# aurelienwaite/SparkNet

Hardware: AMD Instinct MI355X
Metric: images/sec AlexNet training (227x227) at 1/2/4/8 MI355X; scaling efficiency (higher is better)
Workload: dtype bf16; 1 GPU; model=caffenet (bvlc_reference_caffenet / AlexNet), global_batch=256, per_gpu_batch=256, parallelism=dp1, algorithm=local SGD, tau=50, RCCL all-reduce weight averaging, hipgraph=True, streams=3, feed_group=2, fused_input_fold=True, fp8_layers=0, fp8_wgrad=False

## Files before the change

### csrc/kernels/softmax.hip

```cpp
#include "common.h"

#define FLT_MIN_ 1.175494351e-38f

__global__ void softmax_xent_fwd(const bf16_t* __restrict__ x, const float* __restrict__ labels,
                                 float* __restrict__ prob, float* __restrict__ row_loss, float* __restrict__ row_valid,
                                 int M, int C, int has_ignore, int ignore_label) {
  const int lane = threadIdx.x & 63;
  const int row = blockIdx.x * (blockDim.x >> 6) + (threadIdx.x >> 6);
  if (row >= M) return;
  const bf16_t* xr = x + (long long)row * C;
  float m = -INFINITY;
  for (int c = lane; c < C; c += 64) m = fmaxf(m, bf2f(xr[c]));
  m = wave_max(m);
  float s = 0.f;
  for (int c = lane; c < C; c += 64) s += __expf(bf2f(xr[c]) - m);
  s = wave_sum(s);
  const float inv = 1.f / s;
  float* pr = prob + (long long)row * C;
  for (int c = lane; c < C; c += 64) pr[c] = __expf(bf2f(xr[c]) - m) * inv;
  if (lane == 0) {
    int lab = (int)labels[row];
    bool valid = !(has_ignore && lab == ignore_label);
    float nll = 0.f;
    if (valid) {
      float p = __expf(bf2f(xr[min(max(lab, 0), C - 1)]) - m) * inv;
      nll = -__logf(fmaxf(p, FLT_MIN_));
    }
    row_loss[row] = nll;
    row_valid[row] = valid ? 1.f : 0.f;
  }
}

__global__ void xent_reduce(const float* __restrict__ row_loss, const float* __restrict__ row_valid, int M,
                            int normalize, float outer_num, float* __restrict__ out_loss, float* __restrict__ out_norm) {
  __shared__ float ls[16], vs[16];
  float l = 0.f, v = 0.f;
  for (int i = threadIdx.x; i < M; i += blockDim.x) {
    l += row_loss[i];
    v += row_valid[i];
  }
  l = wave_sum(l);
  v = wave_sum(v);
  if ((threadIdx.x & 63) == 0) {
    ls[threadIdx.x >> 6] = l;
    vs[threadIdx.x >> 6] = v;
  }
  __syncthreads();
// ... 4 lines not shown
    norm = fmaxf(norm, 1.f);
    out_loss[0] = L / norm;
    out_norm[0] = norm;
  }
}

extern "C" int sn_softmax_xent_fwd(const bf16_t* x, const float* labels, float* prob, float* row_loss,
                                   float* row_valid, float* out_loss, float* out_norm, long long M, long long C,
                                   long long has_ignore, long long ignore_label, long long normalize,
                                   long long outer_num, hipStream_t st) {
  const int rows_per_block = 4;
  hipLaunchKernelGGL(softmax_xent_fwd, dim3((unsigned)((M + rows_per_block - 1) / rows_per_block)), dim3(256), 0, st, x,
                     labels, prob, row_loss, row_valid, (int)M, (int)C, (int)has_ignore, (int)ignore_label);
  hipLaunchKernelGGL(xent_reduce, dim3(1), dim3(1024), 0, st, row_loss, row_valid, (int)M, (int)normalize,
                     (float)outer_num, out_loss, out_norm);
  return SN_CHECK_LAUNCH();
}

__global__ void softmax_xent_bwd(const float* __restrict__ prob, const float* __restrict__ labels,
                                 const float* __restrict__ loss_weight, const float* __restrict__ norm,
                                 bf16_t* __restrict__ dx, int M, int C, int has_ignore, int ignore_label) {
  const long long total = (long long)M * C;
  const float scale = loss_weight[0] / norm[0];
  for (long long i = blockIdx.x * (long long)blockDim.x + threadIdx.x; i < total; i += (long long)gridDim.x * blockDim.x) {
    const int row = (int)(i / C), c = (int)(i - (long long)row * C);
    const int lab = (int)labels[row];
    float g = 0.f;
    if (!(has_ignore && lab == ignore_label)) g = (prob[i] - (c == lab ? 1.f : 0.f)) * scale;
    dx[i] = f2bf(g);
  }
// ... 78 lines not shown
```

### csrc/kernels/solver.hip

```cpp
#include "common.h"

enum { H_LR = 0, H_MOM, H_WD, H_CLIP, H_NORM, H_DELTA, H_MOM2, H_RMS, H_CORR, H_T, H_SUMSQ = 15 };

SN_DEV void chunk_grad(const float* __restrict__ g, long long o, const long long* __restrict__ src, int cid, int i,
                       float* G) {
  const long long sp = src ? src[4 * cid] : 0;
  if (sp == 0) {
    const float4 gv = *reinterpret_cast<const float4*>(g + o);
    G[0] = gv.x; G[1] = gv.y; G[2] = gv.z; G[3] = gv.w;
    return;
  }
  const float* sl = reinterpret_cast<const float*>(sp);
  const long long ss = src[4 * cid + 1], es = src[4 * cid + 3];
  const int splits = (int)src[4 * cid + 2];
  G[0] = G[1] = G[2] = G[3] = 0.f;
  if (splits >= 16) {
    if (es == 1) {
      const float* p = sl + i;
      for (int l = 0; l < 16; ++l) {
        float P[4] = {0.f, 0.f, 0.f, 0.f};
        int s = l;
        for (; s + 48 < splits; s += 64) {
          float4 v[4];
#pragma unroll
// ... 187 lines not shown
  dim3 grid((unsigned)(grid_limit > 0 && grid_limit < nchunks ? grid_limit : nchunks));
  bool sh = shadow != nullptr;
  const int n = (int)nchunks;
  switch (kind) {
    case 0: launch_kind<0>(l1, clip, sh, grid, st, w, g, h0, h1, shadow, chunk_pos, chunk_mult, hyper, n, chunk_src); break;
    case 1: launch_kind<1>(l1, clip, sh, grid, st, w, g, h0, h1, shadow, chunk_pos, chunk_mult, hyper, n, chunk_src); break;
    case 2: launch_kind<2>(l1, clip, sh, grid, st, w, g, h0, h1, shadow, chunk_pos, chunk_mult, hyper, n, chunk_src); break;
    case 3: launch_kind<3>(l1, clip, sh, grid, st, w, g, h0, h1, shadow, chunk_pos, chunk_mult, hyper, n, chunk_src); break;
    case 4: launch_kind<4>(l1, clip, sh, grid, st, w, g, h0, h1, shadow, chunk_pos, chunk_mult, hyper, n, chunk_src); break;
    case 5: launch_kind<5>(l1, clip, sh, grid, st, w, g, h0, h1, shadow, chunk_pos, chunk_mult, hyper, n, chunk_src); break;
    default: return 8;
  }
  return SN_CHECK_LAUNCH();
}

__global__ void scale_shadow(float* __restrict__ w, bf16_t* __restrict__ shadow, long long n, long long n4,
                             float scale) {
  const long long stride = (long long)gridDim.x * blockDim.x;
  for (long long i = blockIdx.x * (long long)blockDim.x + threadIdx.x; i < n4; i += stride) {
    float4 v = reinterpret_cast<float4*>(w)[i];
    v.x *= scale; v.y *= scale; v.z *= scale; v.w *= scale;
    reinterpret_cast<float4*>(w)[i] = v;
    if (shadow) reinterpret_cast<uint2*>(shadow)[i] = make_uint2(pack2(v.x, v.y), pack2(v.z, v.w));
  }
  for (long long i = 4 * n4 + blockIdx.x * (long long)blockDim.x + threadIdx.x; i < n; i += stride) {
    const float v = w[i] * scale;
    w[i] = v;
    if (shadow) shadow[i] = f2bf(v);
  }
}
// ... 10 lines not shown
```

### sparknet_amd/core/net.py

```python
from __future__ import annotations

import logging
from dataclasses import dataclass, field

import torch

from .. import ops, proto
from .blob import Blob
from .filler import fill
from .layer import Layer, Param, create_layer

log = logging.getLogger("sparknet_amd.net")

PARAM_ALIGN = 64


@dataclass
class NetContext:
    device: torch.device
    dtype: torch.dtype
    phase: int
    seed: int = 1701
    gen: torch.Generator = field(default=None)
    rng_state: torch.Tensor = field(default=None)
# ... 367 lines not shown
            elif prev is not None and prev.numel() == p.count:
                p.data.copy_(prev.reshape(p.shape).to(dev))
        for p in self.params:
            if p.owner is not None:
                r = p.owner
                p.offset = r.offset
                p.data = r.data.view(p.shape)
                p.diff = r.diff.view(p.shape)
                p.compute = r.compute.view(p.shape)
        self.sync_compute()

    def sync_compute(self) -> None:
        if self.flat_compute is not self.flat_data and self.flat_data is not None:
            from .. import ops
            ops.cast_f32_to_bf16(self.flat_data, self.flat_compute)

    def param_segments(self) -> list[tuple[int, int, float, float]]:
        return [(p.offset, p.count, p.lr_mult, p.decay_mult) for p in self.learnable_params]

    def forward_from_to(self, start: int, end: int):
        with ops.precision(self.dtype):
            for li in range(start, end + 1):
                layer = self.layers[li]
                layer.forward(self.bottom_vecs[li], self.top_vecs[li])
                if self.debug_info:
                    self._debug_forward(li)
            return self.loss_value()

    def loss_value(self):
        loss = None
# ... 9 lines not shown

    def forward(self, bottom: list[torch.Tensor] | None = None):
        if bottom is not None:
            for bid, t in zip(self.input_blob_ids, bottom):
                self.blobs[bid].set_nchw(t)
        return self.forward_from_to(0, len(self.layers) - 1)

    def prefill_loss_diffs(self) -> None:
        done = self.__dict__.setdefault("_loss_diff_filled", {})
        for t, w in self._loss_tops:
            d = t.diff
            key = (id(d), d.data_ptr(), d._version, w)
            if done.get(id(t)) != key:
                d.fill_(w)
                done[id(t)] = (id(d), d.data_ptr(), d._version, w)

    def backward_from_to(self, start: int, end: int) -> None:
        self.prefill_loss_diffs()
        for hook in self.pre_backward_hooks:
            hook()
        with ops.precision(self.dtype):
            for li in range(start, end - 1, -1):
                if self.layer_need_backward[li]:
                    self.layers[li].backward(self.top_vecs[li], self.bottom_need_backward[li],
                                             self.bottom_vecs[li])
                    if self.debug_info:
                        self._debug_backward(li)
                for hook in self.backward_hooks:
                    hook(li)

# ... 261 lines not shown
```

### sparknet_amd/core/solver.py

```python
from __future__ import annotations

import logging
import math
import os
import time
from typing import Callable

import numpy as np
import torch

from .. import proto
from .net import Net, blob_proto_to_tensor

log = logging.getLogger("sparknet_amd.solver")

SOLVER_KINDS = {"SGD": 0, "Nesterov": 1, "AdaGrad": 2, "RMSProp": 3, "AdaDelta": 4, "Adam": 5}
_LEGACY_TYPES = {0: "SGD", 1: "Nesterov", 2: "AdaGrad", 3: "RMSProp", 4: "AdaDelta", 5: "Adam"}
N_HISTORY = {"SGD": 1, "Nesterov": 1, "AdaGrad": 1, "RMSProp": 1, "AdaDelta": 2, "Adam": 2}

H_LR, H_MOM, H_WD, H_CLIP, H_NORM, H_DELTA, H_MOM2, H_RMS, H_CORR, H_T = range(10)
N_HYPER = 16


class Solver:
# ... 184 lines not shown
                final[p.offset] = min(final.get(p.offset, wl), wl)
        groups: dict = {}
        for off, li in final.items():
            if off not in late:
                groups.setdefault(li, []).append(seg_of[off])
        big = {li: segs for li, segs in groups.items() if sum(sg[1] for sg in segs) >= min_group}
        rest = [seg_of[o] for o in seg_of if not any(o == sg[0] for segs in big.values() for sg in segs)]
        return big, rest

    def update_params_segments(self, tables, grid_limit: int = 0) -> None:
        from .. import ops
        net = self.net
        ops.solver_update(SOLVER_KINDS[self.type], net.flat_data, net.flat_diff, self.history,
                          net.flat_compute if net.flat_compute is not net.flat_data else None,
                          tables, self.hyper, self.param.regularization_type == "L1", False, grid_limit)

    def update_params(self) -> None:
        from .. import ops
        l1 = self.param.regularization_type == "L1"
        if self.param.regularization_type not in ("L1", "L2"):
            raise ValueError(f"Unknown regularization type: {self.param.regularization_type}")
        net = self.net
        if getattr(self, "slab_tables_dirty", False):
            assert not torch.cuda.is_current_stream_capturing(), "split-K slab layout changed during capture"
            self._build_tables()
        ops.solver_update(SOLVER_KINDS[self.type], net.flat_data, net.flat_diff, self.history,
                          net.flat_compute if net.flat_compute is not net.flat_data else None,
                          self._tables, self.hyper, l1, self.param.clip_gradients > 0)

    def iteration(self):
        net = self.net
        if getattr(self, "fused_offsets", None) or getattr(self, "slab_sinks", None):
            self.stage_hyper()
        net.clear_param_diffs(lazy=True)
        for cb in self.callbacks:
            getattr(cb, "on_start", lambda: None)()
        loss = None
        for _ in range(max(1, self.param.iter_size)):
            l = net.forward_backward()
            loss = l if loss is None else loss + l
            from .. import ops
            ops.advance_rng(net.ctx.rng_state)
        net.finish_param_diffs()
# ... 158 lines not shown
```

### sparknet_amd/engine.py

```python
from __future__ import annotations

import gc
import logging
import os
import time

import torch

from . import ops
from .core.solver import Solver
from .utils import features
from .utils.trace import trace_range

from .ops.spec import ConvSpec

log = logging.getLogger("sparknet_amd.engine")


def fuse_relu(net) -> int:
    if net.device.type == "cuda" and net.dtype == torch.float32:
        return 0
    n = 0
    for li in range(1, len(net.layers)):
        relu = net.layers[li]
# ... 319 lines not shown
        for p in layer.params:
            users[p.offset] = users.get(p.offset, 0) + 1
    flags = (1 if solver.type == "Nesterov" else 0) | (2 if solver.param.regularization_type == "L1" else 0)
    offsets = []
    for li, layer in enumerate(net.layers):
        if layer.type_name != "InnerProduct" or not net.layer_need_backward[li] or not layer.param_grads_needed(0):
            continue
        p = layer.weight
        if p.owner is not None or users.get(p.offset, 0) != 1 or layer.N % 8 or layer.Kdim % 8:
            continue
        layer.fused_update = _FusedFCUpdate(solver, p, flags)
        offsets.append(p.offset)
    if offsets:
        solver.set_fused_update(offsets)
    return len(offsets)


class _SlabGrad:

    def __init__(self, solver, layer):
        self.solver, self.layer = solver, layer
        self.buf = None
        self.desc = None
        self.got = False
        self.table = None

    def begin(self):
        self.got = False

    def end(self):
# ... 415 lines not shown
    def __init__(self, solver: Solver, warmup: int = 2, pre=None, overlap: bool = True, fuse_fc: bool = True,
                 streams: int = 2, comm=None):
        self.solver = solver
        self.pre = pre
        self.comm = comm
        self.graph = None
        self.loss = None
        self.warmup = warmup
        self.overlap = None
        if overlap and solver.overlap_eligible():
            self.overlap = OverlappedUpdate(solver)
            solver.net.backward_hooks.append(self.overlap.hook)
        elif fuse_fc:
            fuse_fc_updates(solver)
            fuse_splitk_updates(solver)
        self.n_streams = streams if not solver.net.debug_info else 1
        self.branches = None
        self._use_branches = False

    def _body(self):
        s = self.solver
        net = s.net
        net.clear_param_diffs(lazy=True)
        for cb in s.callbacks:
            getattr(cb, "on_start", lambda: None)()
        if self.overlap is not None:
            self.overlap.begin()
        if self._use_branches and self.branches is None:
            self.branches = branch_streams(net, self.n_streams) or False
        loss = (self.branches.forward_backward() if self._use_branches and self.branches
                else net.forward_backward())
        net.finish_param_diffs()
        fp8_step(net)
        for cb in s.callbacks:
            getattr(cb, "on_gradients_ready", lambda: None)()
        ops.advance_rng(net.ctx.rng_state)
        if self.overlap is not None:
            self.overlap.end()
        else:
            s.update_params()
        return loss

    def capture(self) -> None:
        s = self.solver
        dev = s.device
        side = torch.cuda.Stream(dev)
        side.wait_stream(torch.cuda.current_stream(dev))
        with torch.cuda.stream(side):
            for w in range(self.warmup):
                self._use_branches = w > 0
# ... 25 lines not shown

    def step(self):
        s = self.solver
        if self.graph is None:
            self.capture()
            return self.loss
        d = self.max_ahead
        if d > 0:
            ring = self.__dict__.setdefault("_ahead", [None] * d)
            k = self.__dict__.get("_ahead_k", 0)
            if ring[k % d] is not None:
                ring[k % d].synchronize()
        if self.pre:
            self.pre()
        s.stage_hyper()
        self.graph.replay()
        s.iter += 1
        if d > 0:
            ev = ring[k % d] or torch.cuda.Event()
            ev.record()
            ring[k % d] = ev
            self._ahead_k = k + 1
        return self.loss


class LocalSGDTrainer:

    def __init__(self, solver: Solver, comm=None, tau: int = 50, feeder=None, use_graph: bool = True,
                 log_every: int = 0, overlap_update: bool = False, fuse_fc: bool = True, streams: int = 2):
        self.solver = solver
# ... 51 lines not shown
```

### sparknet_amd/layers/loss.py

```python
from __future__ import annotations

import torch

from .. import ops
from ..core.layer import Layer, register


def _prod(dims) -> int:
    n = 1
    for d in dims:
        n *= int(d)
    return n


def rows_view(blob, axis, diff=False):
    t = blob.diff if diff else blob.data
    axis = blob.canonical_axis(axis)
    if blob.is_image:
        if axis == 1:
            return t.reshape(-1, blob.shape[1])
        t = _lh().nhwc_to_nchw(t) if t.is_cuda else t.permute(0, 3, 1, 2)
    elif axis == len(blob.shape) - 1 or blob.count_range(axis + 1) == 1:
        return t.reshape(-1, blob.shape[axis])
    outer, A, inner = _prod(blob.shape[:axis]), blob.shape[axis], _prod(blob.shape[axis + 1:])
# ... 87 lines not shown
        self.ignore_label = lp.ignore_label if lp.HasField("ignore_label") else None
        self.normalize = lp.normalize
        self.axis = bottoms[0].canonical_axis(self.lp.softmax_param.axis)

    def reshape(self, bottoms, tops):
        tops[0].reshape((), torch.float32)
        b = bottoms[0]
        outer = b.count_range(0, self.axis)
        inner = b.count_range(self.axis + 1)
        if outer * inner != bottoms[1].count:
            raise ValueError("Number of labels must match number of predictions")
        self.outer = outer
        if len(tops) > 1:
            tops[1].reshape(b.shape, self.dtype)

    def forward(self, bottoms, tops):
        x2 = rows_view(bottoms[0], self.axis)
        loss, prob, norm = ops.softmax_loss_forward(x2, bottoms[1].data, self.ignore_label,
                                                    self.normalize, self.outer)
        self.prob, self.norm = prob, norm
        tops[0].data = loss.reshape(())
        if len(tops) > 1:
            tops[1].data = rows_view_back(prob, bottoms[0], self.axis).to(self.dtype)

    def backward(self, tops, propagate_down, bottoms):
        if len(propagate_down) > 1 and propagate_down[1]:
            raise ValueError("SoftmaxWithLoss cannot backpropagate to label inputs")
        if propagate_down[0]:
            g = ops.softmax_loss_backward(self.prob, bottoms[1].data, tops[0].diff, self.norm,
                                          self.ignore_label, bottoms[0].dtype)
            bottoms[0].diff = rows_view_back(g, bottoms[0], self.axis).to(bottoms[0].dtype)


@register("Softmax")
class SoftmaxLayer(Layer):
    exact_bottoms = 1
    exact_tops = 1

    def layer_setup(self, bottoms, tops):
        self.axis = bottoms[0].canonical_axis(self.lp.softmax_param.axis)

    def reshape(self, bottoms, tops):
        tops[0].reshape(bottoms[0].shape, self.dtype)

    def forward(self, bottoms, tops):
# ... 248 lines not shown
```

### sparknet_amd/layers/vision.py

```python
from __future__ import annotations

import torch

from .. import ops, proto
from ..core.layer import Layer, register
from ..ops.spec import POOL_AVE, POOL_MAX, POOL_STOCHASTIC, ConvSpec, PoolSpec


def _conv_hw(cp, name, rep_name, h_name, w_name, default):
    if cp.HasField(h_name) or cp.HasField(w_name):
        return int(getattr(cp, h_name)), int(getattr(cp, w_name))
    rep = list(getattr(cp, rep_name))
    if len(rep) == 0:
        return default, default
    if len(rep) == 1:
        return int(rep[0]), int(rep[0])
    return int(rep[0]), int(rep[1])


def conv_geometry(cp):
    if cp.HasField("kernel_h") or cp.HasField("kernel_w"):
        kh, kw = cp.kernel_h, cp.kernel_w
    else:
        ks = list(cp.kernel_size)
# ... 173 lines not shown
            if propagate_down[i]:
                _store_logical(b, ops.conv_nd_forward(dtop, w, None, sc), diff=True)


@register("Convolution")
class ConvolutionLayer(Layer):
    exact_bottoms = -1
    min_bottoms = 1
    min_tops = 1

    fuse_relu = False
    relu_gate = False
    folded_input = None
    concat_slot = None
    flipped_weights = None

    def layer_setup(self, bottoms, tops):
        cp = self.lp.convolution_param
        if conv_nd_mode(cp, bottoms[0]):
            self.__class__ = ConvolutionNdLayer
            return self.layer_setup(bottoms, tops)
        if len(bottoms) != len(tops):
            raise ValueError("Convolution needs as many tops as bottoms")
        b = bottoms[0]
        self.R, self.S, self.sh, self.sw, self.ph, self.pw = conv_geometry(cp)
        self.K = int(cp.num_output)
        self.groups = int(cp.group)
        C = b.shape[1]
        if C % self.groups or self.K % self.groups:
            raise ValueError("channels and num_output must be divisible by group")
# ... 14 lines not shown
        if C != self.C:
            raise ValueError(f"{self.name}: input channels changed {self.C} -> {C}")
        return ConvSpec(N, H, W, C, self.K, self.R, self.S, self.sh, self.sw, self.ph, self.pw,
                        1, 1, self.groups)

    def reshape(self, bottoms, tops):
        for b, t in zip(bottoms, tops):
            s = self.spec(b)
            t.reshape((s.N, s.K, s.P, s.Q), self.dtype)

    def forward(self, bottoms, tops):
        w = self.weight.compute
        bias = self.bias.data if self.bias is not None else None
        from ..ops.hip import ConvScratch
        self._ws = [ConvScratch() for _ in bottoms]
        for i, (b, t) in enumerate(zip(bottoms, tops)):
            s = self.spec(b)
            side = self._fp8_out_side(s) if i == 0 else None
            if side is not None:
                from ..ops import gemm as _gemm
                with _gemm.fp8_side_output(side):
                    if self.fp8_slots is not None:
                        t.data = self._forward_fp8(b.data, w, bias, s, out=side.base)
                    else:
                        t.data = ops.conv_forward(b.data, w, bias, s, relu=self.fuse_relu, ws=self._ws[i],
                                                  folded=self.folded_input, out=side.base)
                self.fp8_out[0]._fp8_x_side = side
                continue
            if self.fp8_slots is not None and b.data.is_cuda:
                t.data = self._forward_fp8(b.data, w, bias, s)
# ... 71 lines not shown
            gate = b.data if self.relu_gate else None
            ws = self._ws[i] if i < len(getattr(self, "_ws", ())) else ConvScratch()
            ws.wt = self.flipped_weights
            if self.fp8_dgrad_slots is not None and t.diff.is_cuda:
                dy_side, self._fp8_dy_side = self._fp8_dy_side, None
                ws.fp8_dgrad = Fp8Dgrad(self.ctx.fp8, *self.fp8_dgrad_slots, dy_side)
                xq, self._fp8_xq = self._fp8_xq, None
                if self.fp8_wgrad and xq is not None and dw is not None and i == 0:
                    ws.fp8_wgrad = Fp8Wgrad(self.ctx.fp8, self.fp8_slots[0], xq, self.fp8_dgrad_slots[0])
            if i == 0 and self.fp8_dx_out is not None and propagate_down[i] and self._fp8_ready():
                prod, idy = self.fp8_dx_out
                ws.fp8_dx_side = (self.ctx.fp8.slot(idy), self.ctx.fp8.is_e5m2(idy),
                                  self._side_part("bwd", t.diff.device))
            dw_acc = not (dw is not None and self.grad_overwrite(0))
            db_acc = not (db is not None and self.grad_overwrite(1))
            sink = getattr(self, "slab_grad", None)
            if sink is not None and dw is not None and not dw_acc and not (db is not None and db_acc):
                from ..ops import gemm as _gemm
                with _gemm.defer_reduce(sink):
                    dx = ops.conv_backward(t.diff, b.data, w, s, bool(propagate_down[i]), dw, db, gate, ws,
                                           dw_acc=dw_acc, db_acc=db_acc)
                sink.apply()
            else:
                if sink is not None:
                    sink.begin()
                    sink.end()
                dx = ops.conv_backward(t.diff, b.data, w, s, bool(propagate_down[i]), dw, db, gate, ws,
                                       dw_acc=dw_acc, db_acc=db_acc)
            side, ws.fp8_dx_side_out = ws.fp8_dx_side_out, None
            if side is not None:
# ... 452 lines not shown
```

### sparknet_amd/ops/hip.py

```python
from __future__ import annotations

import contextlib
import ctypes as C
import dataclasses
import os
from typing import NamedTuple

import torch

from . import _lib
from ..utils import features
from .gemm import (EPI_BF16, EPI_F32, EPI_F32_ACC, ConvGeom, Dense, FlipW, Fp8Side, Im2col, colsum, fp8_side_output,
                   gemm, linear_dgrad, linear_fwd, linear_wgrad, side_bytes)
from .spec import POOL_MAX, ConvNdSpec, ConvSpec, PoolSpec

call = _lib.call
BF16 = torch.bfloat16
DGRAD_INPLACE_WEIGHTS = False


def _c(t: torch.Tensor) -> torch.Tensor:
    return t if t.is_contiguous() else t.contiguous()


# ... 124 lines not shown
                         folded[n0:n1] if folded is not None else None, out=y[n0:n1])
        if ws is not None and folded is not None:
            ws.s2d_full = (x.data_ptr(), x._version, folded)
        return y
    ldx = chan_stride(x)
    if not (ldx and _slice_ok(s)):
        x, ldx = _c(x), s.C
    assert x.dtype == BF16 and w.dtype == BF16, (x.dtype, w.dtype)
    if out is not None:
        ldo = chan_stride(out)
        assert (out.is_contiguous() or _slice_ok(s)) and ldo and tuple(out.shape) == (s.N, s.P, s.Q, s.K) \
            and out.dtype == BF16, "conv output slice needs an ungrouped implicit conv and an NHWC channel-slice view"
    plan = _s2d_plan(s)
    if plan is not None:
        f, cp, rf, sf, s2 = plan
        w2 = torch.empty((s.K, rf, sf, s2.C), dtype=BF16, device=x.device)
        call("s2d_weight", _c(w), w2, s.K, s.R, s.S, s.C, f, cp, rf, sf)
        x2 = folded if folded is not None else _s2d_input(x, s, plan)
        if ws is not None:
            ws.s2d = (x.data_ptr(), x._version, x2)
        return conv_forward(x2, w2, b, s2, relu, out=out)
    M = s.N * s.P * s.Q
    if out is not None:
        y, ldy = out, chan_stride(out)
    else:
        y, ldy = torch.empty((s.N, s.P, s.Q, s.K), dtype=BF16, device=x.device), s.K
    if ldx == s.C and ldy == s.K and x.is_contiguous() and packed3x3k64_ok(s):
        from . import gemm as G
        side = G._SIDE if _side_covers(y) else None
        if side is None or not side.e5m2:
            q = (None, None, None)
            if side is not None:
# ... 137 lines not shown
        return bool(getattr(self.dy_side, "only", False))


class Fp8Wgrad(NamedTuple):
    scales: object
    x_slot: int
    xq: torch.Tensor
    dy_slot: int


@dataclasses.dataclass
class ConvScratch:
    s2d: tuple | None = None
    s2d_full: tuple | None = None
    wt: torch.Tensor | None = None
    fp8_dgrad: Fp8Dgrad | None = None
    fp8_wgrad: Fp8Wgrad | None = None
    fp8_dx_side: tuple | None = None
    fp8_dx_side_out: object = None

    def release(self) -> None:
        self.__init__()


class FlipBatch:

    def __init__(self, items, device):
        self.items = list(items)
        self.device = torch.device(device)
        self._build()
# ... 90 lines not shown
    if ((dw is not None or db is not None) and plan is None and ldd == s.K and ldx == s.C and depthwise_ok(s)
            and _dw_io_ok(dy2, x)):
        part, n = _dw_part(s, x.device)
        call("conv_dw_wgrad", dy2, x, part, n, dw, 0 if dw is None else 1 + int(dw_acc),
             db, 0 if db is None else 1 + int(db_acc), s.N, s.H, s.W, s.C, s.sh, s.sw, s.ph, s.pw)
        return
    if db is not None and not fused_db:
        assert ldd == s.K
        colsum(dy2, db, accumulate=db_acc)
    if dw is not None and plan is not None:
        f, cp, rf, sf, s2 = plan
        x2 = _s2d_cached(ws.s2d, x)
        if x2 is None:
            x2 = _s2d_input(x, s, plan)
        k2 = rf * sf * s2.C
        dw2 = torch.empty((s.K, k2), dtype=torch.float32, device=x.device)
        gemm(s.K, k2, M, Dense(dy2, s.K, kcontig=False), Im2col(x2, _geom(s2), kcontig=False), dw2, k2,
             epi=EPI_F32, bias_grad=db if fused_db else None, bias_acc=db_acc)
        call("s2d_weight_grad", dw2, dw, s.K, s.R, s.S, s.C, f, cp, rf, sf, int(dw_acc))
        dw = None
    if dw is not None:
        if _wgrad_implicit_ok(s):
            A = Dense(dy2, ldd, kcontig=False, gstride=s.Kg)
            B = Im2col(x, _geom(s, ldx), kcontig=False, gstride=s.Cg)
            gemm(s.Kg, kred, M, A, B, dw, kred, epi=EPI_F32_ACC if dw_acc else EPI_F32, groups=s.groups,
                 c_gstride=s.Kg * kred, bias_grad=db if fused_db else None, bias_acc=db_acc)
        else:
            kpad = _round8(kred)
            kgp = _round8(s.Kg)
            dw2 = dw.view(s.K, kred)
            for g in range(s.groups):
                col = _im2col(x, s, g, kpad)
                dyg = dy2[:, g * s.Kg:(g + 1) * s.Kg]
                dyg = _c(dyg) if kgp == s.Kg else _pad_cols(dyg, kgp)
# ... 472 lines not shown

def softmax_loss_forward(x2, labels, ignore_label=None, normalize=True, outer_num=None):
    x2 = as_bf16(x2)
    M, Cn = x2.shape
    dev = x2.device
    prob = torch.empty((M, Cn), dtype=torch.float32, device=dev)
    rows = torch.empty((2, M), dtype=torch.float32, device=dev)
    out = torch.empty(2, dtype=torch.float32, device=dev)
    lab = _c(labels.reshape(-1).float())
    call("softmax_xent_fwd", x2, lab, prob, rows[0], rows[1], out[0:1], out[1:2], M, Cn,
         int(ignore_label is not None), int(ignore_label or 0), int(normalize),
         int(outer_num if outer_num is not None else M))
    return out[0], prob, out[1:2]


def softmax_loss_backward(prob, labels, loss_weight, norm, ignore_label=None, dtype=BF16):
    M, Cn = prob.shape
    dx = torch.empty((M, Cn), dtype=BF16, device=prob.device)
    lw = loss_weight.reshape(-1).float()
    call("softmax_xent_bwd", prob, _c(labels.reshape(-1).float()), lw, norm, dx, M, Cn,
         int(ignore_label is not None), int(ignore_label or 0))
    return dx if dtype == BF16 else dx.to(dtype)


def softmax_forward(x2):
    x2 = as_bf16(x2)
    y = torch.empty_like(x2)
    call("softmax_fwd", x2, y, x2.shape[0], x2.shape[1])
    return y

# ... 42 lines not shown
        "src": (torch.tensor(src, dtype=torch.int64, device=device) if slab_chunks and src else None),
        "n": len(pos),
        "part": torch.empty(nparts, dtype=torch.float32, device=device),
        "total": total,
    }


def solver_update(kind, data, diff, history, compute, tables, hyper, l1, clip, grid_limit=0):
    h0 = history[0]
    h1 = history[1] if len(history) > 1 else history[0]
    call("solver_update", int(kind), data, diff, h0, h1, compute, tables["pos"], tables["mult"], tables["n"],
         hyper, int(l1), int(clip), tables["part"], tables["part"].numel(), tables["total"], int(grid_limit),
         tables.get("src"))


def scale_shadow(flat, shadow, scale: float):
    call("scale_shadow", flat, shadow, flat.numel(), float(scale))



def s2d_plan(s: ConvSpec):
    return _s2d_plan(s)


def _labels(labels, label_out):
    if labels is None:
        return None, None
    assert labels.dtype == torch.int32 and label_out.dtype == torch.float32 and label_out.numel() == labels.numel()
    return _c(labels), label_out

# ... 102 lines not shown
```

### sparknet_amd/parallel/comm.py

```python
from __future__ import annotations

import atexit
import datetime
import os
import sys
import threading

import torch
import torch.distributed as dist

DEFAULT_BUCKET_BYTES = 256 << 20
AVERAGE_BUCKET_BYTES = 64 << 20
WATCHDOG_EXIT_CODE = 75



def _scale(flat: torch.Tensor, shadow, scale: float) -> None:
    if flat.is_cuda:
        from ..ops import hip
        hip.scale_shadow(flat, shadow, scale)
    else:
        flat.mul_(scale)
        if shadow is not None:
            shadow.copy_(flat)
# ... 118 lines not shown
        scale = 1.0 / self.world_size
        cuda = flat.is_cuda
        shadow = net.flat_compute if cuda and net.flat_compute is not net.flat_data else None
        ranges = self.bucket_ranges(flat.numel(), bucket_bytes or self.average_bucket_bytes)
        works, t = [], []
        for s, e in ranges:
            t0 = time.perf_counter()
            works.append(self.allreduce_sum(flat[s:e], async_op=True) or ())
            t.append(1e3 * (time.perf_counter() - t0))
        for (s, e), ws in zip(ranges, works):
            for w in ws:
                w.wait()
            _scale(flat[s:e], shadow[s:e] if shadow is not None else None, scale)
        if not cuda:
            net.sync_compute()
        return t

    def allreduce_grads(self, net, average: bool = True) -> None:
        if not self.active:
            return
        self.allreduce_sum(net.flat_diff)
        if average:
            _scale(net.flat_diff, None, 1.0 / self.world_size)

    def allreduce_scores(self, scores: list[float], device=None) -> list[float]:
        if not self.active:
            return list(scores)
        t = torch.tensor(list(scores), dtype=torch.float64 if device is None else torch.float32,
                         device=device or "cpu")
        if device is None and dist.get_backend() == "nccl":
# ... 102 lines not shown
```

### sparknet_amd/utils/features.py

```python
from __future__ import annotations

import os

DEFAULTS = {
    "fuse_pool_lrn": True,
    "fuse_lrn_pool_bwd": True,
    "zero_copy_concat": True,
    "fuse_dropout": True,
    "fuse_fp8_quant": True,
    "fuse_bn_scale": True,
    "branch_depfree": True,
    "fuse_splitk": False,
    "conv_direct_c64": True,
    "conv_direct_k96": True,
    "conv_direct96": True,
    "conv_packed": True,
    "conv_packed44": True,
    "conv_packed11": False,
    "conv_packed_k64": True,
    "conv_direct_fp8": True,
    "conv_depthwise": True,
    "fp8_wgrad_bias": True,
    "fp8_side_frag": True,
    "fp8_dx_only": True,
}

_cache: tuple[str, dict] = ("", {})
# ... 21 lines not shown
```

Measured before the change: 120,400 images/sec.

## Fuse softmax loss fwd/bwd and fold loss reduction into solver tail kernel

Adds a fused softmax-cross-entropy kernel that computes probabilities, per-row loss and the input gradient in one pass, with the loss reduction deferred. A new solver tail kernel performs the SGD/Nesterov update, runs the loss reduction in block 0, and scatters updated weights directly into the space-to-depth folded (and optionally flipped) bf16 weight copies through index maps. The first-layer convolution then reuses those pre-folded weights and gradient buffers instead of re-folding each step. Together these remove several small launches and the separate weight fold/unfold passes, at the cost of gather/scatter through maps, staleness tracking via weight stamps, and extra coupling between forward, backward and solver.

```diff
diff --git a/csrc/kernels/loss_sum.h b/csrc/kernels/loss_sum.h
--- /dev/null
+++ b/csrc/kernels/loss_sum.h
@@ -0,0 +1,31 @@
+#pragma once
+#include "common.h"
+
+SN_DEV void xent_reduce_block256(const float* __restrict__ row_loss, const float* __restrict__ row_valid, int M,
+                                 int normalize, float outer_num, float* __restrict__ out_loss,
+                                 float* __restrict__ out_norm, float* ls, float* vs) {
+#pragma unroll
+  for (int q = 0; q < 4; ++q) {
+    const int v = threadIdx.x + 256 * q;
+    float l = 0.f, s = 0.f;
+    for (int i = v; i < M; i += 1024) {
+      l += row_loss[i];
+      s += row_valid[i];
+    }
+    l = wave_sum(l);
+    s = wave_sum(s);
+    if ((threadIdx.x & 63) == 0) {
+      ls[v >> 6] = l;
+      vs[v >> 6] = s;
+    }
+  }
+  __syncthreads();
+  if (threadIdx.x == 0) {
+    float L = 0.f, V = 0.f;
+    for (int w = 0; w < 16; ++w) { L += ls[w]; V += vs[w]; }
+    float norm = normalize ? V : outer_num;
+    norm = fmaxf(norm, 1.f);
+    out_loss[0] = L / norm;
+    out_norm[0] = norm;
+  }
+}
diff --git a/csrc/kernels/softmax.hip b/csrc/kernels/softmax.hip
--- a/csrc/kernels/softmax.hip
+++ b/csrc/kernels/softmax.hip
@@ -31,6 +31,39 @@
   }
 }
 
+__global__ void softmax_xent_fwd_bwd(const bf16_t* __restrict__ x, const float* __restrict__ labels,
+                                     float* __restrict__ prob, float* __restrict__ row_loss,
+                                     float* __restrict__ row_valid,
+                                     const float* __restrict__ loss_weight, float norm, bf16_t* __restrict__ dx,
+                                     int M, int C) {
+  const int lane = threadIdx.x & 63;
+  const int row = blockIdx.x * (blockDim.x >> 6) + (threadIdx.x >> 6);
+  if (row >= M) return;
+  const bf16_t* xr = x + (long long)row * C;
+  float m = -INFINITY;
+  for (int c = lane; c < C; c += 64) m = fmaxf(m, bf2f(xr[c]));
+  m = wave_max(m);
+  float s = 0.f;
+  for (int c = lane; c < C; c += 64) s += __expf(bf2f(xr[c]) - m);
+  s = wave_sum(s);
+  const float inv = 1.f / s;
+  float* pr = prob + (long long)row * C;
+  bf16_t* dr = dx + (long long)row * C;
+  const int lab = (int)labels[row];
+  const float scale = loss_weight[0] / norm;
+  for (int c = lane; c < C; c += 64) {
+#pragma clang fp contract(off)
+    const float p = __expf(bf2f(xr[c]) - m) * inv;
+    pr[c] = p;
+    dr[c] = f2bf((p - (c == lab ? 1.f : 0.f)) * scale);
+  }
+  if (lane == 0) {
+    const float p = __expf(bf2f(xr[min(max(lab, 0), C - 1)]) - m) * inv;
+    row_loss[row] = -__logf(fmaxf(p, FLT_MIN_));
+    row_valid[row] = 1.f;
+  }
+}
+
 __global__ void xent_reduce(const float* __restrict__ row_loss, const float* __restrict__ row_valid, int M,
                             int normalize, float outer_num, float* __restrict__ out_loss, float* __restrict__ out_norm) {
   __shared__ float ls[16], vs[16];
@@ -65,6 +98,20 @@
                      labels, prob, row_loss, row_valid, (int)M, (int)C, (int)has_ignore, (int)ignore_label);
   hipLaunchKernelGGL(xent_reduce, dim3(1), dim3(1024), 0, st, row_loss, row_valid, (int)M, (int)normalize,
                      (float)outer_num, out_loss, out_norm);
+  return SN_CHECK_LAUNCH();
+}
+
+extern "C" int sn_softmax_xent_fwd_bwd(const bf16_t* x, const float* labels, float* prob, float* row_loss,
+                                       float* row_valid, float* out_loss, float* out_norm, const float* loss_weight,
+                                       bf16_t* dx, long long M, long long C, long long normalize, long long outer_num,
+                                       long long reduce, hipStream_t st) {
+  const int rows_per_block = 4;
+  const float norm = fmaxf((float)(normalize ? M : outer_num), 1.f);
+  hipLaunchKernelGGL(softmax_xent_fwd_bwd, dim3((unsigned)((M + rows_per_block - 1) / rows_per_block)), dim3(256), 0,
+                     st, x, labels, prob, row_loss, row_valid, loss_weight, norm, dx, (int)M, (int)C);
+  if (reduce)
+    hipLaunchKernelGGL(xent_reduce, dim3(1), dim3(1024), 0, st, row_loss, row_valid, (int)M, (int)normalize,
+                       (float)outer_num, out_loss, out_norm);
   return SN_CHECK_LAUNCH();
 }
 
diff --git a/csrc/kernels/solver.hip b/csrc/kernels/solver.hip
--- a/csrc/kernels/solver.hip
+++ b/csrc/kernels/solver.hip
@@ -1,4 +1,5 @@
 #include "common.h"
+#include "loss_sum.h"
 
 enum { H_LR = 0, H_MOM, H_WD, H_CLIP, H_NORM, H_DELTA, H_MOM2, H_RMS, H_CORR, H_T, H_SUMSQ = 15 };
 
@@ -225,6 +226,100 @@
   return SN_CHECK_LAUNCH();
 }
 
+template <int KIND, bool L1>
+__global__ void __launch_bounds__(256) solver_tail_kernel(float* __restrict__ w, const float* __restrict__ g,
+                                                          float* __restrict__ h0, bf16_t* __restrict__ shadow,
+                                                          const long long* __restrict__ chunk_pos,
+                                                          const float* __restrict__ chunk_mult,
+                                                          const float* __restrict__ hyper, int nchunks,
+                                                          const long long* __restrict__ ext, long long* rng,
+                                                          const float* __restrict__ row_loss,
+                                                          const float* __restrict__ row_valid, int M, int normalize,
+                                                          float outer_num, float* __restrict__ out_loss,
+                                                          float* __restrict__ out_norm) {
+  __shared__ float ls[16], vs[16];
+  if (blockIdx.x == 0) {
+    if (rng != nullptr && threadIdx.x == 0) rng[1] += 1;
+    if (row_loss != nullptr) xent_reduce_block256(row_loss, row_valid, M, normalize, outer_num, out_loss, out_norm, ls, vs);
+  }
+  for (int cid = blockIdx.x; cid < nchunks; cid += gridDim.x) {
+  const long long start = chunk_pos[2 * cid];
+  const int count = (int)chunk_pos[2 * cid + 1];
+  const float lr_mult = chunk_mult[2 * cid], decay_mult = chunk_mult[2 * cid + 1];
+  const float rate = hyper[H_LR] * lr_mult;
+  const float mom = hyper[H_MOM];
+  const float decay = hyper[H_WD] * decay_mult;
+  const float gscale = hyper[H_NORM];
+  const float* gsrc = reinterpret_cast<const float*>(ext[4 * cid]);
+  const int* gmap = reinterpret_cast<const int*>(ext[4 * cid + 1]);
+  bf16_t* sdst = reinterpret_cast<bf16_t*>(ext[4 * cid + 2]);
+  const int* smap = reinterpret_cast<const int*>(ext[4 * cid + 3]);
+  for (int i = threadIdx.x * 4; i < count; i += blockDim.x * 4) {
+    const long long o = start + i;
+    float4 wv = *reinterpret_cast<float4*>(w + o);
+    float G[4];
+    if (gsrc == nullptr) {
+      const float4 gv = *reinterpret_cast<const float4*>(g + o);
+      G[0] = gv.x; G[1] = gv.y; G[2] = gv.z; G[3] = gv.w;
+    } else {
+      const int4 gi = *reinterpret_cast<const int4*>(gmap + i);
+      const int I[4] = {gi.x, gi.y, gi.z, gi.w};
+#pragma unroll
+      for (int k = 0; k < 4; ++k) G[k] = I[k] >= 0 ? gsrc[I[k]] : g[o + k];
+    }
+    float4 a = *reinterpret_cast<float4*>(h0 + o);
+    float W[4] = {wv.x, wv.y, wv.z, wv.w};
+    float A[4] = {a.x, a.y, a.z, a.w};
+#pragma unroll
+    for (int k = 0; k < 4; ++k) {
+      float gg = G[k] * gscale;
+      gg += decay * (L1 ? ((W[k] > 0.f) - (W[k] < 0.f)) : W[k]);
+      float upd;
+      if (KIND == 0) {
+        A[k] = mom * A[k] + rate * gg;
+        upd = A[k];
+      } else {
+        float prev = A[k];
+        A[k] = mom * A[k] + rate * gg;
+        upd = (1.f + mom) * A[k] - mom * prev;
+      }
+      W[k] -= upd;
+    }
+    *reinterpret_cast<float4*>(w + o) = make_float4(W[0], W[1], W[2], W[3]);
+    *reinterpret_cast<float4*>(h0 + o) = make_float4(A[0], A[1], A[2], A[3]);
+    *reinterpret_cast<uint2*>(shadow + o) = make_uint2(pack2(W[0], W[1]), pack2(W[2], W[3]));
+    if (sdst != nullptr) {
+      const int4 si = *reinterpret_cast<const int4*>(smap + i);
+      const int I[4] = {si.x, si.y, si.z, si.w};
+#pragma unroll
+      for (int k = 0; k < 4; ++k)
+        if (I[k] >= 0) sdst[I[k]] = f2bf(W[k]);
+    }
+  }
+  }
+}
+
+extern "C" int sn_solver_tail(long long kind, float* w, const float* g, float* h0, bf16_t* shadow,
+                              const long long* chunk_pos, const float* chunk_mult, long long nchunks,
+                              const float* hyper, long long l1, const long long* ext, long long* rng,
+                              const float* row_loss, const float* row_valid, long long M, long long normalize,
+                              long long outer_num, float* out_loss, float* out_norm, hipStream_t st) {
+  if (shadow == nullptr || ext == nullptr || (kind != 0 && kind != 1)) return 8;
+  dim3 grid((unsigned)(nchunks > 0 ? nchunks : 1));
+  const int n = (int)(nchunks > 0 ? nchunks : 0);
+#define SN_TAIL(KIND, L1)                                                                                       \
+  hipLaunchKernelGGL((solver_tail_kernel<KIND, L1>), grid, dim3(256), 0, st, w, g, h0, shadow, chunk_pos,       \
+                     chunk_mult, hyper, n, ext, rng, row_loss, row_valid, (int)M, (int)normalize,               \
+                     (float)outer_num, out_loss, out_norm)
+  if (kind == 0) {
+    if (l1) SN_TAIL(0, true); else SN_TAIL(0, false);
+  } else {
+    if (l1) SN_TAIL(1, true); else SN_TAIL(1, false);
+  }
+#undef SN_TAIL
+  return SN_CHECK_LAUNCH();
+}
+
 __global__ void scale_shadow(float* __restrict__ w, bf16_t* __restrict__ shadow, long long n, long long n4,
                              float scale) {
   const long long stride = (long long)gridDim.x * blockDim.x;
diff --git a/sparknet_amd/core/net.py b/sparknet_amd/core/net.py
--- a/sparknet_amd/core/net.py
+++ b/sparknet_amd/core/net.py
@@ -405,6 +405,16 @@
         if self.flat_compute is not self.flat_data and self.flat_data is not None:
             from .. import ops
             ops.cast_f32_to_bf16(self.flat_data, self.flat_compute)
+        self.weights_changed()
+
+    weights_epoch = 0
+
+    def weights_changed(self) -> None:
+        self.weights_epoch += 1
+
+    def weights_stamp(self) -> tuple:
+        return (self.weights_epoch, self.flat_data._version if self.flat_data is not None else 0,
+                self.flat_compute._version if self.flat_compute is not None else 0)
 
     def param_segments(self) -> list[tuple[int, int, float, float]]:
         return [(p.offset, p.count, p.lr_mult, p.decay_mult) for p in self.learnable_params]
@@ -444,6 +454,15 @@
             if done.get(id(t)) != key:
                 d.fill_(w)
                 done[id(t)] = (id(d), d.data_ptr(), d._version, w)
+
+    def constant_loss_diff(self, top):
+        done = self.__dict__.get("_loss_diff_filled", {})
+        for t, w in self._loss_tops:
+            if t is top and t.has_diff():
+                d = t.diff
+                if done.get(id(t)) == (id(d), d.data_ptr(), d._version, w):
+                    return d
+        return None
 
     def backward_from_to(self, start: int, end: int) -> None:
         self.prefill_loss_diffs()
diff --git a/sparknet_amd/core/solver.py b/sparknet_amd/core/solver.py
--- a/sparknet_amd/core/solver.py
+++ b/sparknet_amd/core/solver.py
@@ -222,6 +222,7 @@
         ops.solver_update(SOLVER_KINDS[self.type], net.flat_data, net.flat_diff, self.history,
                           net.flat_compute if net.flat_compute is not net.flat_data else None,
                           tables, self.hyper, self.param.regularization_type == "L1", False, grid_limit)
+        net.weights_changed()
 
     def update_params(self) -> None:
         from .. import ops
@@ -235,6 +236,7 @@
         ops.solver_update(SOLVER_KINDS[self.type], net.flat_data, net.flat_diff, self.history,
                           net.flat_compute if net.flat_compute is not net.flat_data else None,
                           self._tables, self.hyper, l1, self.param.clip_gradients > 0)
+        net.weights_changed()
 
     def iteration(self):
         net = self.net
diff --git a/sparknet_amd/engine.py b/sparknet_amd/engine.py
--- a/sparknet_amd/engine.py
+++ b/sparknet_amd/engine.py
@@ -357,6 +357,186 @@
     if offsets:
         solver.set_fused_update(offsets)
     return len(offsets)
+
+
+class _LossHead:
+
+    def __init__(self, net):
+        self.net = net
+        self.armed = False
+        self.defer_to = None
+        self.pending = None
+
+    def constant_weight(self, top):
+        return self.net.constant_loss_diff(top)
+
+    def take_sum(self, layer) -> bool:
+        return self.armed and self.defer_to is layer
+
+
+def fuse_loss_head(net):
+    if (net.device.type != "cuda" or net.dtype == torch.float32 or net.debug_info
+            or not features.enabled("fuse_loss_head")):
+        return None
+    head = getattr(net, "_loss_head", None)
+    if head is None:
+        heads = [layer for li, layer in enumerate(net.layers)
+                 if layer.type_name == "SoftmaxWithLoss" and net.layer_need_backward[li]
+                 and net.bottom_need_backward[li][0]]
+        if not heads:
+            return None
+        head = net._loss_head = _LossHead(net)
+        for layer in heads:
+            layer.loss_head = head
+    return head
+
+
+class _TailCopies:
+
+    def __init__(self, tail, w2, dw2):
+        self.tail, self.w2, self.dw2 = tail, w2, dw2
+
+    def armed(self) -> bool:
+        return self.tail.armed
+
+
+class SolverTail:
+
+    def __init__(self, solver, head, plan):
+        self.solver, self.head = solver, head
+        self.folds, self.flip_batch, self.extras = plan
+        self.armed = False
+        self.stamp = None
+        self.refreshes = 0
+        self._build()
+        net = solver.net
+        if self.flip_batch is not None:
+            hooks = net.pre_backward_hooks
+            hooks[hooks.index(self.flip_batch.run)] = self._flip_unless_armed
+        for layer, w2, dw2, _ in self.folds:
+            layer.tail_copies = _TailCopies(self, w2, dw2)
+
+    @staticmethod
+    def plan(solver):
+        from .ops import hip
+        net = solver.net
+        if (net.device.type != "cuda" or net.dtype == torch.float32 or net.debug_info
+                or not features.enabled("solver_tail") or not solver.overlap_eligible()
+                or solver.type not in ("SGD", "Nesterov") or solver.param.regularization_type not in ("L1", "L2")
+                or net.flat_compute is net.flat_data or getattr(solver, "slab_sinks", None)):
+            return None
+        users: dict = {}
+        for layer in net.layers:
+            for p in layer.params:
+                users[p.offset] = users.get(p.offset, 0) + 1
+        fused = set(getattr(solver, "fused_offsets", ()))
+
+        def own(p):
+            return (p.owner is None and users.get(p.offset, 0) == 1 and p.offset not in fused
+                    and p.compute.data_ptr() == net.flat_compute.data_ptr() + 2 * p.offset and p.compute.is_contiguous())
+
+        folds, extras = [], {}
+        for li, layer in enumerate(net.layers):
+            if layer.type_name != "Convolution":
+                continue
+            s = layer.spec(net.bottom_vecs[li][0])
+            fp = hip.s2d_plan(s)
+            if fp is None:
+                continue
+            if len(net.bottom_vecs[li]) != 1 or not own(layer.weight) or hip._image_chunk(s) < s.N:
+                return None
+            f, cp, rf, sf, s2 = fp
+            w2 = torch.zeros((s.K, rf, sf, s2.C), dtype=torch.bfloat16, device=net.device)
+            dw2 = None
+            if (net.layer_need_backward[li] and layer.param_grads_needed(0) and s.Kg % 8 == 0
+                    and net._overwrite_ok().get(layer.weight.offset, False)):
+                dw2 = torch.empty((s.K, rf * sf * s2.C), dtype=torch.float32, device=net.device)
+            folds.append((layer, w2, dw2, s))
+            extras[layer.weight.offset] = (hip.s2d_unfold_map(s), dw2, w2)
+        fb = getattr(net, "_flip_batch", None) if features.enabled("solver_tail_flips") else None
+        if fb is not None:
+            if fb.run not in net.pre_backward_hooks:
+                return None
+            by_wt = {layer.flipped_weights.data_ptr(): layer for layer in net.layers
+                     if getattr(layer, "flipped_weights", None) is not None}
+            for w, wt, G, Kg, R, S, Cg in fb.items:
+                layer = by_wt.get(wt.data_ptr())
+                if layer is None or not own(layer.weight) or layer.weight.offset in extras:
+                    return None
+                extras[layer.weight.offset] = (hip.flip_map(G, Kg, R, S, Cg), None, wt)
+        return folds, fb, extras
+
+    def _build(self) -> None:
+        from .ops import hip
+        s = self.solver
+        fused = set(getattr(s, "fused_offsets", ()))
+        segs = [sg for sg in s.net.param_segments() if sg[0] not in fused]
+        self.tables = hip.solver_tail_tables(segs, s.net.num_param_elems, s.device, self.extras)
+        self._fused = fused
+
+    def _flip_unless_armed(self) -> None:
+        if not self.armed:
+            self.flip_batch.run()
+
+    def stale(self) -> bool:
+        return self.stamp != self.solver.net.weights_stamp()
+
+    def refresh(self) -> None:
+        from .ops import hip
+        for layer, w2, _, s in self.folds:
+            f, cp, rf, sf, _ = hip.s2d_plan(s)
+            hip.call("s2d_weight", layer.weight.compute, w2, s.K, s.R, s.S, s.C, f, cp, rf, sf)
+        if self.flip_batch is not None:
+            self.flip_batch.run()
+        self.stamp = self.solver.net.weights_stamp()
+        self.refreshes += 1
+
+    def begin(self) -> None:
+        if ([x.data_ptr() for x in self.tables["held"]] != self.tables["ptrs"]
+                or set(getattr(self.solver, "fused_offsets", ())) != self._fused):
+            assert not torch.cuda.is_current_stream_capturing(), "solver tail tables changed during capture"
+            self._build()
+        if self.stale():
+            self.refresh()
+        self.armed = True
+        self.head_armed(True)
+
+    def head_armed(self, on: bool) -> None:
+        if self.head is not None:
+            self.head.armed = on
+            if not on:
+                self.head.pending = None
+
+    def run(self) -> None:
+        from .ops import hip
+        from .core.solver import SOLVER_KINDS
+        s, net = self.solver, self.solver.net
+        loss = self.head.pending if self.head is not None else None
+        hip.solver_tail(SOLVER_KINDS[s.type], net.flat_data, net.flat_diff, s.history, net.flat_compute, self.tables,
+                        s.hyper, s.param.regularization_type == "L1", net.ctx.rng_state, loss)
+        self.armed = False
+        self.head_armed(False)
+        self.stamp = net.weights_stamp()
+
+    def abort(self) -> None:
+        self.armed = False
+        self.head_armed(False)
+        self.stamp = None
+
+
+def solver_tail(solver):
+    plan = SolverTail.plan(solver)
+    if plan is None:
+        return None
+    head = fuse_loss_head(solver.net)
+    if head is not None:
+        net = solver.net
+        tops = net._loss_tops
+        heads = [(li, layer) for li, layer in enumerate(net.layers) if getattr(layer, "loss_head", None) is head] \
+            if len(tops) == 1 and tops[0][1] == 1.0 else []
+        if len(heads) == 1 and net.top_vecs[heads[0][0]][0] is tops[0][0]:
+            head.defer_to = heads[0][1]
+    return SolverTail(solver, head, plan)
 
 
 class _SlabGrad:
@@ -802,6 +982,9 @@
         elif fuse_fc:
             fuse_fc_updates(solver)
             fuse_splitk_updates(solver)
+        self.tail = solver_tail(solver) if (fuse_fc and self.overlap is None) else None
+        if self.tail is None and features.enabled("loss_head_without_tail"):
+            fuse_loss_head(solver.net)
         self.n_streams = streams if not solver.net.debug_info else 1
         self.branches = None
         self._use_branches = False
@@ -816,12 +999,23 @@
             self.overlap.begin()
         if self._use_branches and self.branches is None:
             self.branches = branch_streams(net, self.n_streams) or False
-        loss = (self.branches.forward_backward() if self._use_branches and self.branches
-                else net.forward_backward())
-        net.finish_param_diffs()
-        fp8_step(net)
-        for cb in s.callbacks:
-            getattr(cb, "on_gradients_ready", lambda: None)()
+        tail = self.tail
+        if tail is not None:
+            tail.begin()
+        try:
+            loss = (self.branches.forward_backward() if self._use_branches and self.branches
+                    else net.forward_backward())
+            net.finish_param_diffs()
+            fp8_step(net)
+            for cb in s.callbacks:
+                getattr(cb, "on_gradients_ready", lambda: None)()
+            if tail is not None:
+                tail.run()
+                return loss
+        except BaseException:
+            if tail is not None:
+                tail.abort()
+            raise
         ops.advance_rng(net.ctx.rng_state)
         if self.overlap is not None:
             self.overlap.end()
@@ -877,6 +1071,8 @@
         if self.pre:
             self.pre()
         s.stage_hyper()
+        if self.tail is not None and self.tail.stale():
+            self.tail.refresh()
         self.graph.replay()
         s.iter += 1
         if d > 0:
diff --git a/sparknet_amd/layers/loss.py b/sparknet_amd/layers/loss.py
--- a/sparknet_amd/layers/loss.py
+++ b/sparknet_amd/layers/loss.py
@@ -125,8 +125,28 @@
         if len(tops) > 1:
             tops[1].reshape(b.shape, self.dtype)
 
+    loss_head = None
+    _dx = None
+
     def forward(self, bottoms, tops):
         x2 = rows_view(bottoms[0], self.axis)
+        self._dx = None
+        head = self.loss_head
+        if head is not None and x2.is_cuda:
+            lw = head.constant_weight(tops[0])
+            from ..ops import hip
+            if hip.loss_head_norm(x2.shape[0], self.outer, self.ignore_label, self.normalize, lw is not None) is not None:
+                defer = head.take_sum(self)
+                loss, prob, norm, dx, rows = hip.softmax_loss_forward_backward(
+                    x2, bottoms[1].data, lw, self.normalize, self.outer, reduce=not defer)
+                if defer:
+                    head.pending = (rows, x2.shape[0], bool(self.normalize), self.outer, loss, norm)
+                self._dx = (dx, lw, lw._version)
+                self.prob, self.norm = prob, norm
+                tops[0].data = loss.reshape(())
+                if len(tops) > 1:
+                    tops[1].data = rows_view_back(prob, bottoms[0], self.axis).to(self.dtype)
+                return
         loss, prob, norm = ops.softmax_loss_forward(x2, bottoms[1].data, self.ignore_label,
                                                     self.normalize, self.outer)
         self.prob, self.norm = prob, norm
@@ -137,9 +157,13 @@
     def backward(self, tops, propagate_down, bottoms):
         if len(propagate_down) > 1 and propagate_down[1]:
             raise ValueError("SoftmaxWithLoss cannot backpropagate to label inputs")
+        fused, self._dx = self._dx, None
         if propagate_down[0]:
-            g = ops.softmax_loss_backward(self.prob, bottoms[1].data, tops[0].diff, self.norm,
-                                          self.ignore_label, bottoms[0].dtype)
+            if fused is not None and tops[0].diff is fused[1] and fused[1]._version == fused[2]:
+                g = fused[0]
+            else:
+                g = ops.softmax_loss_backward(self.prob, bottoms[1].data, tops[0].diff, self.norm,
+                                              self.ignore_label, bottoms[0].dtype)
             bottoms[0].diff = rows_view_back(g, bottoms[0], self.axis).to(bottoms[0].dtype)
 
 
diff --git a/sparknet_amd/layers/vision.py b/sparknet_amd/layers/vision.py
--- a/sparknet_amd/layers/vision.py
+++ b/sparknet_amd/layers/vision.py
@@ -211,6 +211,7 @@
     folded_input = None
     concat_slot = None
     flipped_weights = None
+    tail_copies = None
 
     def layer_setup(self, bottoms, tops):
         cp = self.lp.convolution_param
@@ -255,6 +256,9 @@
         bias = self.bias.data if self.bias is not None else None
         from ..ops.hip import ConvScratch
         self._ws = [ConvScratch() for _ in bottoms]
+        tc = self.tail_copies
+        if tc is not None and tc.armed():
+            self._ws[0].w2 = tc.w2
         for i, (b, t) in enumerate(zip(bottoms, tops)):
             s = self.spec(b)
             side = self._fp8_out_side(s) if i == 0 else None
@@ -356,6 +360,12 @@
                                   self._side_part("bwd", t.diff.device))
             dw_acc = not (dw is not None and self.grad_overwrite(0))
             db_acc = not (db is not None and self.grad_overwrite(1))
+            tc = self.tail_copies
+            if tc is not None and tc.dw2 is not None and tc.armed():
+                if dw is None or dw_acc or len(bottoms) != 1:
+                    raise RuntimeError(f"{self.name}: the solver tail reads this layer's folded weight gradient, "
+                                       "which must be written once per step")
+                ws.dw2 = tc.dw2
             sink = getattr(self, "slab_grad", None)
             if sink is not None and dw is not None and not dw_acc and not (db is not None and db_acc):
                 from ..ops import gemm as _gemm
diff --git a/sparknet_amd/ops/hip.py b/sparknet_amd/ops/hip.py
--- a/sparknet_amd/ops/hip.py
+++ b/sparknet_amd/ops/hip.py
@@ -162,8 +162,12 @@
     plan = _s2d_plan(s)
     if plan is not None:
         f, cp, rf, sf, s2 = plan
-        w2 = torch.empty((s.K, rf, sf, s2.C), dtype=BF16, device=x.device)
-        call("s2d_weight", _c(w), w2, s.K, s.R, s.S, s.C, f, cp, rf, sf)
+        w2 = ws.w2 if ws is not None else None
+        if w2 is None:
+            w2 = torch.empty((s.K, rf, sf, s2.C), dtype=BF16, device=x.device)
+            call("s2d_weight", _c(w), w2, s.K, s.R, s.S, s.C, f, cp, rf, sf)
+        else:
+            assert tuple(w2.shape) == (s.K, rf, sf, s2.C) and w2.dtype == BF16 and w2.is_contiguous()
         x2 = folded if folded is not None else _s2d_input(x, s, plan)
         if ws is not None:
             ws.s2d = (x.data_ptr(), x._version, x2)
@@ -331,6 +335,8 @@
     s2d: tuple | None = None
     s2d_full: tuple | None = None
     wt: torch.Tensor | None = None
+    w2: torch.Tensor | None = None
+    dw2: torch.Tensor | None = None
     fp8_dgrad: Fp8Dgrad | None = None
     fp8_wgrad: Fp8Wgrad | None = None
     fp8_dx_side: tuple | None = None
@@ -451,10 +457,15 @@
         if x2 is None:
             x2 = _s2d_input(x, s, plan)
         k2 = rf * sf * s2.C
-        dw2 = torch.empty((s.K, k2), dtype=torch.float32, device=x.device)
+        keep = ws.dw2
+        if keep is not None:
+            assert not dw_acc, "a folded weight gradient left for the solver tail cannot accumulate"
+            assert tuple(keep.shape) == (s.K, k2) and keep.dtype == torch.float32 and keep.is_contiguous()
+        dw2 = keep if keep is not None else torch.empty((s.K, k2), dtype=torch.float32, device=x.device)
         gemm(s.K, k2, M, Dense(dy2, s.K, kcontig=False), Im2col(x2, _geom(s2), kcontig=False), dw2, k2,
              epi=EPI_F32, bias_grad=db if fused_db else None, bias_acc=db_acc)
-        call("s2d_weight_grad", dw2, dw, s.K, s.R, s.S, s.C, f, cp, rf, sf, int(dw_acc))
+        if keep is None:
+            call("s2d_weight_grad", dw2, dw, s.K, s.R, s.S, s.C, f, cp, rf, sf, int(dw_acc))
         dw = None
     if dw is not None:
         if _wgrad_implicit_ok(s):
@@ -957,6 +968,31 @@
     return out[0], prob, out[1:2]
 
 
+def loss_head_norm(M: int, outer_num, ignore_label, normalize, weight_is_constant: bool):
+    if ignore_label is not None or not weight_is_constant:
+        return None
+    n = int(M) if normalize else int(outer_num if outer_num is not None else M)
+    if not (0 < int(M) < (1 << 24) and n < (1 << 24)):
+        return None
+    return float(max(n, 1))
+
+
+def softmax_loss_forward_backward(x2, labels, loss_weight, normalize=True, outer_num=None, reduce=True):
+    x2 = as_bf16(x2)
+    M, Cn = x2.shape
+    dev = x2.device
+    prob = torch.empty((M, Cn), dtype=torch.float32, device=dev)
+    rows = torch.empty((2, M), dtype=torch.float32, device=dev)
+    out = torch.empty(2, dtype=torch.float32, device=dev)
+    dx = torch.empty((M, Cn), dtype=BF16, device=dev)
+    lab = _c(labels.reshape(-1).float())
+    lw = loss_weight.reshape(-1)
+    assert lw.dtype == torch.float32 and lw.numel() >= 1
+    call("softmax_xent_fwd_bwd", x2, lab, prob, rows[0], rows[1], out[0:1], out[1:2], lw, dx, M, Cn,
+         int(normalize), int(outer_num if outer_num is not None else M), int(reduce))
+    return out[0], prob, out[1:2], dx, rows
+
+
 def softmax_loss_backward(prob, labels, loss_weight, norm, ignore_label=None, dtype=BF16):
     M, Cn = prob.shape
     dx = torch.empty((M, Cn), dtype=BF16, device=prob.device)
@@ -1029,6 +1065,88 @@
          tables.get("src"))
 
 
+def s2d_fold_map(s: ConvSpec) -> torch.Tensor:
+    f, cp, rf, sf, s2 = _s2d_plan(s)
+    c2 = f * f * cp
+    j = torch.arange(s.K * rf * sf * c2, dtype=torch.int64)
+    cc, t = j % c2, j // c2
+    sfi, t = t % sf, t // sf
+    rfi, k = t % rf, t // rf
+    c, d = cc % cp, cc // cp
+    r, ss = rfi * f + d // f, sfi * f + d % f
+    src = ((k * s.R + r) * s.S + ss) * s.C + c
+    return torch.where((r < s.R) & (ss < s.S) & (c < s.C), src, torch.full_like(src, -1)).to(torch.int32)
+
+
+def s2d_unfold_map(s: ConvSpec) -> torch.Tensor:
+    f, cp, rf, sf, s2 = _s2d_plan(s)
+    i = torch.arange(s.K * s.R * s.S * s.C, dtype=torch.int64)
+    c, t = i % s.C, i // s.C
+    ss, t = t % s.S, t // s.S
+    r, k = t % s.R, t // s.R
+    dst = ((k * rf + r // f) * sf + ss // f) * (f * f * cp) + ((r % f) * f + ss % f) * cp + c
+    return dst.to(torch.int32)
+
+
+def flip_map(G: int, Kg: int, R: int, S: int, Cg: int) -> torch.Tensor:
+    rs = R * S
+    i = torch.arange(G * Kg * rs * Cg, dtype=torch.int64)
+    c, t = i % Cg, i // Cg
+    tap, t = t % rs, t // rs
+    k, g = t % Kg, t // Kg
+    return (((g * Cg + c) * rs + (rs - 1 - tap)) * Kg + k).to(torch.int32)
+
+
+MAP_CHUNK = 1024
+
+
+def solver_tail_tables(segments, total: int, device, extras=None) -> dict:
+    extras = extras or {}
+    pos, mult, maps, ext, held, at = [], [], [], [], [], 0
+    for off, cnt, lm, dm in segments:
+        padded = -(-cnt // 64) * 64
+        e = extras.get(off)
+        if e is None:
+            for s in range(0, padded, CHUNK):
+                pos.append((off + s, min(CHUNK, padded - s)))
+                mult.append((lm, dm))
+                ext.append((None, 0, None, 0))
+            continue
+        m, gsrc, sdst = e
+        assert m.dtype == torch.int32 and m.numel() == cnt and int(m.min()) >= 0
+        for tsr, dt in ((gsrc, torch.float32), (sdst, BF16)):
+            assert tsr is None or (tsr.is_contiguous() and tsr.dtype == dt and int(m.max()) < tsr.numel())
+        mp = torch.full((padded,), -1, dtype=torch.int32)
+        mp[:cnt] = m
+        maps.append(mp)
+        for s in range(0, padded, MAP_CHUNK):
+            pos.append((off + s, min(MAP_CHUNK, padded - s)))
+            mult.append((lm, dm))
+            ext.append((gsrc, at + s, sdst, at + s))
+        at += padded
+        held += [x for x in (gsrc, sdst) if x is not None]
+    t = {"pos": torch.tensor(pos or [(0, 0)], dtype=torch.int64, device=device),
+         "mult": torch.tensor(mult or [(0.0, 0.0)], dtype=torch.float32, device=device),
+         "n": len(pos), "total": total}
+    dev_maps = (torch.cat(maps) if maps else torch.zeros(4, dtype=torch.int32)).to(device)
+    base = dev_maps.data_ptr()
+    rows = [(0 if g is None else g.data_ptr(), 0 if g is None else base + 4 * gm,
+             0 if d is None else d.data_ptr(), 0 if d is None else base + 4 * dm) for g, gm, d, dm in ext]
+    t["ext"] = torch.tensor(rows or [(0, 0, 0, 0)], dtype=torch.int64, device=device)
+    t["maps"] = dev_maps
+    t["held"] = held
+    t["ptrs"] = [x.data_ptr() for x in held]
+    return t
+
+
+def solver_tail(kind, data, diff, history, compute, tables, hyper, l1, rng_state=None, loss=None):
+    assert int(kind) in (0, 1) and compute is not None
+    rows, M, normalize, outer, out_loss, out_norm = loss if loss is not None else (None, 0, False, 0, None, None)
+    call("solver_tail", int(kind), data, diff, history[0], compute, tables["pos"], tables["mult"], tables["n"],
+         hyper, int(l1), tables["ext"], rng_state, None if rows is None else rows[0], None if rows is None else rows[1],
+         int(M), int(bool(normalize)), int(outer if outer is not None else M), out_loss, out_norm)
+
+
 def scale_shadow(flat, shadow, scale: float):
     call("scale_shadow", flat, shadow, flat.numel(), float(scale))
 
diff --git a/sparknet_amd/parallel/comm.py b/sparknet_amd/parallel/comm.py
--- a/sparknet_amd/parallel/comm.py
+++ b/sparknet_amd/parallel/comm.py
@@ -156,6 +156,7 @@
             _scale(flat[s:e], shadow[s:e] if shadow is not None else None, scale)
         if not cuda:
             net.sync_compute()
+        net.weights_changed()
         return t
 
     def allreduce_grads(self, net, average: bool = True) -> None:
diff --git a/sparknet_amd/utils/features.py b/sparknet_amd/utils/features.py
--- a/sparknet_amd/utils/features.py
+++ b/sparknet_amd/utils/features.py
@@ -11,6 +11,10 @@
     "fuse_bn_scale": True,
     "branch_depfree": True,
     "fuse_splitk": False,
+    "fuse_loss_head": True,
+    "loss_head_without_tail": False,
+    "solver_tail": True,
+    "solver_tail_flips": False,
     "conv_direct_c64": True,
     "conv_direct_k96": True,
     "conv_direct96": True,
```

Result: faster. 121,800 images/sec (median of 6 runs) (+1.2%).
